# samrussell/zlib-ng

Measured on AMD Instinct MI355X. Metric: GB/s input throughput (adler32, crc32, deflate lvl6, inflate) @1/2/4/8 GPU vs CPU ref, higher is better.
Workload: dtype u8; 1 GPU; configs[1]: crc32 + adler32 over a 1024 MiB synthetic buffer per GPU, HBM-resident, fused single pass + on-device combine; bytes_per_gpu=1073741824, parallelism=single, rehearsal_same_gpu=False

## Files before the change

zlib-ng_amd/csrc/checksum.hip:

```cpp
#include "checksum_kernel.h"

#include <atomic>

namespace zr {

static std::atomic<int> g_reserved_cus{0};

static int pick_groups(const Context *c, long long nunits) {
    long long g = c->cus - g_reserved_cus.load(std::memory_order_relaxed);
    if (g < 1) g = 1;
    if (g > kMaxGroups) g = kMaxGroups;
    if (nunits < g) g = nunits > 0 ? nunits : 1;
    return (int)g;
}

void checksum_reset_reserved_cus() { g_reserved_cus.store(0, std::memory_order_relaxed); }

int launch_checksum(bool do_adler, bool do_crc, uint32_t adler, uint32_t crc, const void *d_buf, void *d_dst,
                    size_t len, uint32_t *d_out_adler, uint32_t *d_out_crc, hipStream_t stream,
                    const uint32_t *d_seed_adler, const uint32_t *d_seed_crc) {
    Context *c = ctx();
    if (!c) {
        set_error("zng_rocm_init() has not succeeded");
        return ZNG_ROCM_ENODEV;
    }
    DeviceGuard dev;
    if ((!d_buf && len) || (do_adler && !d_out_adler) || (do_crc && !d_out_crc)) {
        set_error("null device pointer");
        return ZNG_ROCM_EINVAL;
    }
    if (len >> 34) {
        set_error("length above 16 GiB per call is not supported");
        return ZNG_ROCM_EINVAL;
    }
    Workspace *ws = workspace_for(stream);
    if (!ws) return ZNG_ROCM_ENOMEM;

    const uintptr_t p = (uintptr_t)d_buf;
    const uintptr_t a0 = p & ~(uintptr_t)15;
    const uintptr_t tail_base = (p + len) & ~(uintptr_t)15;
    const bool copy = d_dst != nullptr;
    if (copy && (((uintptr_t)d_dst ^ p) & 15)) {
        set_error("fold_copy needs src and dst with the same address mod 16");
        return ZNG_ROCM_EINVAL;
    }

    StreamArgs sa;
    sa.a0 = (const uint8_t *)a0;
    sa.dst0 = copy ? (uint8_t *)d_dst - (p - a0) : nullptr;
    sa.n = (long long)len;
    sa.body = (long long)(tail_base - a0);
    sa.nunits = (sa.body + kUnitBytes - 1) / kUnitBytes;
    sa.head = (int)(p - a0);
    sa.tail = (int)((p + len) - tail_base);
    sa.phase_stamps = nullptr;
    for (int k = 0; k < 4; ++k)
        for (int i = 0; i < 8; ++i) {
            sa.bits.stride[k][i] = c->host_tables.stride_tab[k][1u << i];
            sa.bits.x32[k][i] = c->host_tables.x32_tab[k][1u << i];
        }

    FinalArgs fa;
    fa.tail_base = (const uint8_t *)tail_base;
    fa.tail_dst = copy ? (uint8_t *)d_dst + (tail_base - p) : nullptr;
    fa.n = sa.n;
    fa.nunits = sa.nunits;
    fa.tail_lo = sa.body == 0 ? sa.head : 0;
    fa.tail_hi = sa.tail;
    if (len == 0) fa.tail_lo = fa.tail_hi = 0;
    fa.adler_seed = adler;
    fa.crc_seed = crc;
    fa.crc_len_pow = do_crc ? xpow_bytes(c->host_tables.pow_tab, (uint64_t)len) : 0u;
    fa.adler_seed_ptr = d_seed_adler;
    fa.crc_seed_ptr = d_seed_crc;
    fa.do_adler = do_adler;
    fa.do_crc = do_crc;

    const int groups = pick_groups(c, sa.nunits);
    fa.groups = groups;
    if (sa.nunits > 0) {
        dim3 grid(groups), block(kWgThreads);
#define ZR_LAUNCH(A, C, K) \
        ZR_LAUNCH_TRACED((stream_kernel<A, C, K>), grid, block, stream, sa, c->tables, ws->partials)
        if (copy) {
            if (do_adler && do_crc) ZR_LAUNCH(true, true, true);
            else if (do_adler) ZR_LAUNCH(true, false, true);
            else ZR_LAUNCH(false, true, true);
        } else {
            if (do_adler && do_crc) ZR_LAUNCH(true, true, false);
            else if (do_adler) ZR_LAUNCH(true, false, false);
            else ZR_LAUNCH(false, true, false);
        }
#undef ZR_LAUNCH
        ZR_HIP(hipGetLastError());
    } else {
        ZR_HIP(hipMemsetAsync(ws->partials, 0, sizeof(Partial) * groups, stream));
    }
    hipLaunchKernelGGL(finalize_kernel, dim3(1), dim3(256), 0, stream, fa, c->tables, ws->partials,
                       d_out_adler, d_out_crc);
    ZR_HIP(hipGetLastError());
    return ZNG_ROCM_OK;
}

int launch_checksum_batch_device(bool do_adler, bool do_crc, const StreamArgs *d_messages, const FinalArgs *d_finals,
                                 Partial *d_part, size_t rows, uint32_t *d_out2, hipStream_t stream) {
    Context *c = ctx();
    if (!c) return ZNG_ROCM_ENODEV;
    if (!rows) return ZNG_ROCM_OK;
    for (size_t first = 0; first < rows; first += 32768) {
        const size_t n = rows - first < 32768 ? rows - first : 32768;
        dim3 grid(1, (unsigned)n), block(kWgThreads);
        if (do_adler && do_crc)
            ZR_LAUNCH_TRACED((stream_kernel_batch<true, true>), grid, block, stream, d_messages + first, c->tables, d_part + first);
        else if (do_adler)
            ZR_LAUNCH_TRACED((stream_kernel_batch<true, false>), grid, block, stream, d_messages + first, c->tables, d_part + first);
        else
            ZR_LAUNCH_TRACED((stream_kernel_batch<false, true>), grid, block, stream, d_messages + first, c->tables, d_part + first);
        ZR_HIP(hipGetLastError());
        hipLaunchKernelGGL(finalize_kernel_batch, dim3((unsigned)n), dim3(256), 0, stream, d_finals + first, c->tables,
                           d_part + first, d_out2 + 2 * first);
        ZR_HIP(hipGetLastError());
    }
    return ZNG_ROCM_OK;
}

}

using namespace zr;

extern "C" {

int zng_rocm_adler32_dev(uint32_t adler, const void *d_buf, size_t len, uint32_t *d_out, void *stream) {
    return launch_checksum(true, false, adler, 0, d_buf, nullptr, len, d_out, nullptr, (hipStream_t)stream);
}

int zng_rocm_crc32_dev(uint32_t crc, const void *d_buf, size_t len, uint32_t *d_out, void *stream) {
    return launch_checksum(false, true, 0, crc, d_buf, nullptr, len, nullptr, d_out, (hipStream_t)stream);
}

int zng_rocm_adler32_crc32_dev(uint32_t adler, uint32_t crc, const void *d_buf, size_t len, uint32_t *d_out2,
                               void *stream) {
    if (!d_out2) return ZNG_ROCM_EINVAL;
    return launch_checksum(true, true, adler, crc, d_buf, nullptr, len, d_out2, d_out2 + 1, (hipStream_t)stream);
}

int zng_rocm_fold_copy_dev(int which, uint32_t adler, uint32_t crc, void *d_dst, const void *d_src, size_t len,
                           uint32_t *d_out2, void *stream) {
    if (which < 1 || which > 3 || !d_out2 || (!d_dst && len)) return ZNG_ROCM_EINVAL;
    if (len == 0) d_dst = nullptr;
    return launch_checksum((which & 1) != 0, (which & 2) != 0, adler, crc, d_src, d_dst, len, d_out2, d_out2 + 1,
                           (hipStream_t)stream);
}

int zng_rocm_reserve_cus(int n) {
    Context *c = ctx();
    if (!c) {
        set_error("zng_rocm_init() has not succeeded");
        return ZNG_ROCM_ENODEV;
    }
    if (n < 0 || n >= c->cus) return ZNG_ROCM_EINVAL;
    g_reserved_cus.store(n, std::memory_order_relaxed);
    return ZNG_ROCM_OK;
}

int zng_rocm_checksums_dev(int which, const zng_rocm_check_job *jobs, size_t njobs, uint32_t *d_out2, void *stream) {
    Context *c = ctx();
    if (!c) {
        set_error("zng_rocm_init() has not succeeded");
        return ZNG_ROCM_ENODEV;
    }
    if (!njobs) return ZNG_ROCM_OK;
    if (which < 1 || which > 3 || !jobs || !d_out2) return ZNG_ROCM_EINVAL;
    const bool do_adler = (which & 1) != 0, do_crc = (which & 2) != 0;
    hipStream_t st = (hipStream_t)stream;
    DeviceGuard dev;
    Workspace *ws = workspace_for(st);
    if (!ws) return ZNG_ROCM_ENOMEM;
    std::lock_guard<std::mutex> use(ws->mu);
    size_t max_units = 1;
    for (size_t i = 0; i < njobs; ++i) {
        if ((!jobs[i].buf && jobs[i].len) || (jobs[i].len >> 34)) {
            set_error("job %zu: null buffer or more than 16 GiB", i);
            return ZNG_ROCM_EINVAL;
        }
        const size_t u = (size_t)((jobs[i].len + 15 + kUnitBytes) / kUnitBytes);
        if (u > max_units) max_units = u;
    }
    size_t G = (max_units + 1023) / 1024;
    if (G > 16) G = 16;
    constexpr size_t kRows = 32768;
    const size_t per = sizeof(StreamArgs) + sizeof(FinalArgs);
    const size_t rows_max = njobs < kRows ? njobs : kRows;
    uint8_t *d_msg = nullptr, *h_msg = nullptr;
    Partial *d_part = nullptr;
    if (int rc = scratch_reserve(ws, kScrCheckMessages, rows_max * per, false, (void **)&d_msg)) return rc;
    if (int rc = scratch_reserve(ws, kScrCheckPartials, rows_max * G * sizeof(Partial), false, (void **)&d_part)) return rc;
    for (size_t first = 0; first < njobs; first += kRows) {
        const size_t rows = njobs - first < kRows ? njobs - first : kRows;
        if (int rc = host_tables_acquire(ws)) return rc;
        if (int rc = scratch_reserve(ws, kScrCheckMessagesHost, rows_max * per, true, (void **)&h_msg)) return rc;
        StreamArgs *sa = reinterpret_cast<StreamArgs *>(h_msg);
        FinalArgs *fa = reinterpret_cast<FinalArgs *>(h_msg + rows * sizeof(StreamArgs));
        for (size_t r = 0; r < rows; ++r) {
            const zng_rocm_check_job &j = jobs[first + r];
            const uintptr_t p = (uintptr_t)j.buf;
            const uintptr_t a0 = p & ~(uintptr_t)15;
            const uintptr_t tail_base = (p + j.len) & ~(uintptr_t)15;
            StreamArgs &s = sa[r];
            s.a0 = (const uint8_t *)a0;
            s.dst0 = nullptr;
            s.n = (long long)j.len;
            s.body = (long long)(tail_base - a0);
            s.nunits = (s.body + kUnitBytes - 1) / kUnitBytes;
            s.head = (int)(p - a0);
            s.tail = (int)((p + j.len) - tail_base);
            s.phase_stamps = nullptr;
            for (int k = 0; k < 4; ++k)
                for (int i = 0; i < 8; ++i) {
                    s.bits.stride[k][i] = c->host_tables.stride_tab[k][1u << i];
                    s.bits.x32[k][i] = c->host_tables.x32_tab[k][1u << i];
                }
            FinalArgs &f = fa[r];
            f.tail_base = (const uint8_t *)tail_base;
            f.tail_dst = nullptr;
            f.n = s.n;
            f.nunits = s.nunits;
            f.tail_lo = s.body == 0 ? s.head : 0;
            f.tail_hi = s.tail;
            if (j.len == 0) f.tail_lo = f.tail_hi = 0;
            f.groups = (int)G;
            f.adler_seed = j.adler;
            f.crc_seed = j.crc;
            f.crc_len_pow = do_crc ? xpow_bytes(c->host_tables.pow_tab, (uint64_t)j.len) : 0u;
            f.adler_seed_ptr = nullptr;
            f.crc_seed_ptr = nullptr;
            f.do_adler = do_adler;
            f.do_crc = do_crc;
        }
        ZR_HIP(hipMemcpyAsync(d_msg, h_msg, rows * per, hipMemcpyHostToDevice, st));
        if (int rc = host_tables_release(ws, st)) return rc;
        const StreamArgs *d_sa = reinterpret_cast<const StreamArgs *>(d_msg);
        const FinalArgs *d_fa = reinterpret_cast<const FinalArgs *>(d_msg + rows * sizeof(StreamArgs));
        dim3 grid((unsigned)G, (unsigned)rows), block(kWgThreads);
        if (do_adler && do_crc) ZR_LAUNCH_TRACED((stream_kernel_batch<true, true>), grid, block, st, d_sa, c->tables, d_part);
        else if (do_adler) ZR_LAUNCH_TRACED((stream_kernel_batch<true, false>), grid, block, st, d_sa, c->tables, d_part);
        else ZR_LAUNCH_TRACED((stream_kernel_batch<false, true>), grid, block, st, d_sa, c->tables, d_part);
        ZR_HIP(hipGetLastError());
        hipLaunchKernelGGL(finalize_kernel_batch, dim3((unsigned)rows), dim3(256), 0, st, d_fa, c->tables, d_part,
                           d_out2 + 2 * first);
        ZR_HIP(hipGetLastError());
    }
    return ZNG_ROCM_OK;
}

}
```

zlib-ng_amd/csrc/checksum_kernel.h:

```cpp
#pragma once
#include "context.h"
#include "checksum_args.h"

namespace zr {

typedef uint32_t u32x4_t __attribute__((ext_vector_type(4)));

__device__ __forceinline__ void st_stream(uint8_t *p, uint4 v) {
    u32x4_t x = {v.x, v.y, v.z, v.w};
    __builtin_nontemporal_store(x, reinterpret_cast<u32x4_t *>(p));
}

__device__ __forceinline__ uint4 ld_stream(const uint8_t *p) {
#ifdef ZR_EXPERIMENT_PLAIN_LOADS
    const u32x4_t v = *reinterpret_cast<const u32x4_t *>(p);
#else
    const u32x4_t v = __builtin_nontemporal_load(reinterpret_cast<const u32x4_t *>(p));
#endif
    return make_uint4(v.x, v.y, v.z, v.w);
}

__device__ __forceinline__ void lds_barrier() {
    __builtin_amdgcn_fence(__ATOMIC_RELEASE, "workgroup", "local");
    __builtin_amdgcn_s_barrier();
    __builtin_amdgcn_fence(__ATOMIC_ACQUIRE, "workgroup", "local");
}

__device__ __forceinline__ uint4 mask_low_bytes(uint4 v, int k) {
    uint32_t w[4] = {v.x, v.y, v.z, v.w};
#pragma unroll
    for (int i = 0; i < 4; ++i) {
        int kk = k - 4 * i;
        if (kk >= 4) w[i] = 0;
        else if (kk > 0) w[i] &= 0xffffffffu << (8 * kk);
    }
    return make_uint4(w[0], w[1], w[2], w[3]);
}

__device__ __forceinline__ uint32_t braid_step(const uint32_t *lut, uint32_t rep, uint32_t s, uint32_t w) {
    uint32_t r0 = lut[(((s)       & 0xffu) << 5) + rep];
    uint32_t r1 = lut[(1u << 13) + (((s >> 8)  & 0xffu) << 5) + rep];
    uint32_t r2 = lut[(2u << 13) + (((s >> 16) & 0xffu) << 5) + rep];
    uint32_t r3 = lut[(3u << 13) + (((s >> 24)       ) << 5) + rep];
    return r0 ^ r1 ^ r2 ^ r3 ^ w;
}

__device__ __forceinline__ uint32_t xor3(uint32_t a, uint32_t b, uint32_t c) {
    return __builtin_amdgcn_bitop3_b32(a, b, c, 0x96);
}
__device__ __forceinline__ uint32_t and_xor(uint32_t a, uint32_t b, uint32_t c) {
    return __builtin_amdgcn_bitop3_b32(a, b, c, 0x6a);
}

typedef const __attribute__((address_space(3))) uint32_t *lds_u32_ptr;
template <int K>
__device__ __forceinline__ void put_index_byte(uint32_t &addr, uint32_t s) {
    if constexpr (K == 0) asm("v_mov_b32_sdwa %0, %1 dst_sel:BYTE_1 dst_unused:UNUSED_PRESERVE src0_sel:BYTE_0" : "+v"(addr) : "v"(s));
    if constexpr (K == 1) asm("v_mov_b32_sdwa %0, %1 dst_sel:BYTE_1 dst_unused:UNUSED_PRESERVE src0_sel:BYTE_1" : "+v"(addr) : "v"(s));
    if constexpr (K == 2) asm("v_mov_b32_sdwa %0, %1 dst_sel:BYTE_1 dst_unused:UNUSED_PRESERVE src0_sel:BYTE_2" : "+v"(addr) : "v"(s));
    if constexpr (K == 3) asm("v_mov_b32_sdwa %0, %1 dst_sel:BYTE_1 dst_unused:UNUSED_PRESERVE src0_sel:BYTE_3" : "+v"(addr) : "v"(s));
}
struct BraidAddr {
    uint32_t a0, a1, a2, a3;
};
__device__ __forceinline__ uint32_t braid_step_bytes(BraidAddr &A, uint32_t s, uint32_t w) {
    put_index_byte<0>(A.a0, s);
    const uint32_t r0 = *(lds_u32_ptr)(uintptr_t)A.a0;
    put_index_byte<1>(A.a1, s);
    const uint32_t r1 = *(lds_u32_ptr)(uintptr_t)A.a1;
    put_index_byte<2>(A.a2, s);
    const uint32_t r2 = *(lds_u32_ptr)(uintptr_t)A.a2;
    put_index_byte<3>(A.a3, s);
    const uint32_t r3 = *(lds_u32_ptr)(uintptr_t)A.a3;
    return xor3(xor3(r0, r1, r2), r3, w);
}

template <bool XOR>
__device__ __forceinline__ uint32_t wave_reduce(uint32_t v) {
    auto op = [](uint32_t a, uint32_t b) { return XOR ? (a ^ b) : (a + b); };
    v = op(v, (uint32_t)__builtin_amdgcn_mov_dpp((int)v, 0xB1, 0xf, 0xf, true));
    v = op(v, (uint32_t)__builtin_amdgcn_mov_dpp((int)v, 0x4E, 0xf, 0xf, true));
    v = op(v, (uint32_t)__builtin_amdgcn_mov_dpp((int)v, 0x141, 0xf, 0xf, true));
    v = op(v, (uint32_t)__builtin_amdgcn_mov_dpp((int)v, 0x140, 0xf, 0xf, true));
    return op(op((uint32_t)__builtin_amdgcn_readlane((int)v, 0), (uint32_t)__builtin_amdgcn_readlane((int)v, 16)),
              op((uint32_t)__builtin_amdgcn_readlane((int)v, 32), (uint32_t)__builtin_amdgcn_readlane((int)v, 48)));
}

__device__ __forceinline__ uint32_t mul_by_rows(const uint4 *rows, int stride, int idx, uint32_t r) {
    uint32_t acc = 0;
#pragma unroll
    for (int kq = 0; kq < 8; ++kq) {
        const uint4 a = rows[kq * stride + idx];
        acc = and_xor((uint32_t)__builtin_amdgcn_sbfe((int)r, 31 - 4 * kq, 1), a.x, acc);
        acc = and_xor((uint32_t)__builtin_amdgcn_sbfe((int)r, 30 - 4 * kq, 1), a.y, acc);
        acc = and_xor((uint32_t)__builtin_amdgcn_sbfe((int)r, 29 - 4 * kq, 1), a.z, acc);
        acc = and_xor((uint32_t)__builtin_amdgcn_sbfe((int)r, 28 - 4 * kq, 1), a.w, acc);
    }
    return acc;
}

constexpr int kVarBothBuffers = 1;
constexpr int kVarFoldX32     = 2;
constexpr int kVarEarlyPow    = 4;
#ifdef ZR_CRC_VARIANTS
constexpr int kVarNoReplicate = 16;
constexpr int kVarNoMultiply  = 32;
#else
constexpr int kVarNoReplicate = 0, kVarNoMultiply = 0;
#endif
constexpr int kVarBuildTables = 64;
constexpr int kVarLdsBarrier  = 128;
constexpr int kVarByteAddr    = 1024;
constexpr int kVarDirectImage = 2048;
constexpr int kVarTreeEpilogue = 4096;
constexpr int kVarWavePrio    = 8192;
constexpr int kVarEarlyRows   = 768;
constexpr int kCrcVariant = kVarFoldX32 | kVarBuildTables | kVarLdsBarrier | kVarByteAddr | kVarDirectImage | kVarTreeEpilogue;

template <bool DO_ADLER, bool DO_CRC, bool COPY, int V, bool PROFILE, int UNROLL>
__device__ __forceinline__ void stream_body(const StreamArgs &args, const DeviceTables *__restrict__ tabs,
                                            Partial *__restrict__ partials, const long long G, const long long g) {
#ifndef ZR_CRC_VARIANTS
    static_assert(V == kCrcVariant, "the product instantiates the one tuned variant; the others are for tools/micro/crc_phases.hip");
#endif
    __shared__ __attribute__((aligned(65536))) uint32_t lut[DO_CRC ? 4 * 256 * 32 : 32];
    __shared__ uint32_t stage[DO_CRC ? 4 * 256 + 256 + 4 * 256 : 4];
    __shared__ uint32_t red[3][kWgThreads / 64];
    constexpr bool TREE = (V & kVarTreeEpilogue) != 0;
    __shared__ uint4 tree_rows[(DO_CRC && TREE) ? 640 : 1];

    const int t = threadIdx.x;
    const uint32_t rep = t & 31;
    auto stamp = [&](int k) {
        if constexpr (PROFILE) {
            if (t == 0) args.phase_stamps[8 * g + k] = wall_clock64();
        }
    };
    stamp(0);
    if constexpr ((V & kVarWavePrio) != 0) {
        const int wv = __builtin_amdgcn_readfirstlane(t >> 6);
        if (wv >= 12) __builtin_amdgcn_s_setprio(3);
        else if (wv >= 8) __builtin_amdgcn_s_setprio(2);
        else if (wv >= 4) __builtin_amdgcn_s_setprio(1);
    }

    const long long q = args.nunits / G, r = args.nunits % G;
    const long long u_lo = g * q + (g < r ? g : r);
    const long long u_hi = u_lo + q + (g < r ? 1 : 0);

    long long off = args.body - (args.nunits - u_lo) * (long long)kUnitBytes + (long long)t * kPieceBytes;

    const bool head_unit = u_lo < u_hi && u_lo == 0;
    const long long groups = (u_hi - u_lo - (head_unit ? 1 : 0)) / UNROLL;
    const long long gstride = (long long)UNROLL * kUnitBytes;
    uint4 bufA[UNROLL], bufB[UNROLL];
    auto request = [&](uint4 (&buf)[UNROLL], long long at) {
#pragma unroll
        for (int j = 0; j < UNROLL; ++j) buf[j] = ld_stream(args.a0 + at + (long long)j * kUnitBytes);
    };
    const long long first_at = off + (head_unit ? (long long)kUnitBytes : 0ll);
    bool b_requested = false;
    uint32_t group_w0 = 0, group_w1 = 0;
    uint32_t part[32];
    uint4 tree_row = make_uint4(0, 0, 0, 0);
    if constexpr (DO_CRC) {
        const unsigned long long k_after = (unsigned long long)(args.nunits - u_hi);
        if constexpr ((V & kVarBuildTables) != 0) {
            constexpr int early = (V & kVarEarlyRows) == 0 ? UNROLL : ((V & kVarEarlyRows) >> 8) - 1;
            if (groups > 0) {
#pragma unroll
                for (int j = 0; j < early; ++j) bufA[j] = ld_stream(args.a0 + first_at + (long long)j * kUnitBytes);
            }
            if constexpr ((V & kVarBothBuffers) != 0 && early == UNROLL) {
                if (groups > 1) {
                    request(bufB, first_at + gstride);
                    b_requested = true;
                }
            }
            group_w0 = tabs->unit_pow[0][k_after & 1023u];
            group_w1 = tabs->unit_pow[1][(k_after >> 10) & 1023u];
            if constexpr (TREE) tree_row = *reinterpret_cast<const uint4 *>(tabs->tree_pp[t]);
            if constexpr ((V & kVarEarlyPow) != 0) {
#pragma unroll
                for (int k = 0; k < 32; ++k) part[k] = tabs->lane_pow[k][t];
            }
            const int k = __builtin_amdgcn_readfirstlane(t >> 8);
            const uint32_t e = (uint32_t)t & 255u;
            if constexpr ((V & kVarDirectImage) != 0) {
                static_assert((V & kVarDirectImage) == 0 || ((V & kVarByteAddr) != 0 && (V & kVarFoldX32) != 0),
                              "direct image: byte-addressed layout and x^32 fold only");
                uint32_t m[7];
#pragma unroll
                for (int b = 0; b < 7; ++b) m[b] = (uint32_t)__builtin_amdgcn_sbfe((int)((uint32_t)t >> 3), b, 1);
#pragma unroll
                for (int j = 0; j < 4; ++j) {
                    uint32_t v = 0;
#pragma unroll
                    for (int b = 0; b < 7; ++b) v = and_xor(m[b], args.bits.stride[j][b], v);
#pragma unroll
                    for (int h = 0; h < 2; ++h) {
                        const uint32_t vv = h ? v ^ args.bits.stride[j][7] : v;
                        const int slot = (j >> 1) * 512 + ((h * 128 + (t >> 3)) << 1) + (j & 1);
                        reinterpret_cast<uint4 *>(lut)[slot * 8 + (t & 7)] = make_uint4(vv, vv, vv, vv);
                    }
                }
                uint32_t xv = 0;
#pragma unroll
                for (int i = 0; i < 8; ++i) xv = and_xor((uint32_t)__builtin_amdgcn_sbfe((int)e, i, 1), args.bits.x32[k][i], xv);
                stage[1280 + t] = xv;
            } else {
                uint32_t sv = 0, xv = 0;
#pragma unroll
                for (int i = 0; i < 8; ++i) {
                    const uint32_t m = 0u - ((e >> i) & 1u);
                    sv ^= args.bits.stride[k][i] & m;
                    xv ^= args.bits.x32[k][i] & m;
                }
                stage[t] = sv;
                stage[1280 + t] = xv;
                if (t < 256) {
                    uint32_t r = e;
#pragma unroll
                    for (int i = 0; i < 8; ++i) r = (r >> 1) ^ (kCrcPoly & (0u - (r & 1u)));
                    stage[1024 + t] = r;
                }
            }
        } else {
            uint4 tab = make_uint4(0, 0, 0, 0);
            if (t < 256) {
                tab = reinterpret_cast<const uint4 *>(&tabs->stride_tab[0][0])[t];
            } else if (t < 320) {
                tab = reinterpret_cast<const uint4 *>(tabs->byte_tab)[t - 256];
            } else if (t < 576) {
                tab = reinterpret_cast<const uint4 *>(&tabs->x32_tab[0][0])[t - 320];
            }
            group_w0 = tabs->unit_pow[0][k_after & 1023u];
            group_w1 = tabs->unit_pow[1][(k_after >> 10) & 1023u];
            if (groups > 0) request(bufA, first_at);
            if constexpr ((V & kVarBothBuffers) != 0) {
                if (groups > 1) {
                    request(bufB, first_at + gstride);
                    b_requested = true;
                }
            }
            if constexpr ((V & kVarEarlyPow) != 0) {
#pragma unroll
                for (int k = 0; k < 32; ++k) part[k] = tabs->lane_pow[k][t];
            }
            if (t < 576) reinterpret_cast<uint4 *>(stage)[t] = tab;
        }
        if constexpr ((V & kVarDirectImage) == 0) {
            if constexpr ((V & kVarLdsBarrier) != 0) lds_barrier();
            else __syncthreads();
        }
        stamp(1);
        if constexpr ((V & kVarNoReplicate) == 0 && (V & kVarDirectImage) == 0) {
#pragma unroll
            for (int i = 0; i < 8; ++i) {
                const uint32_t v = stage[i * 128 + (t >> 3)];
                if constexpr ((V & kVarByteAddr) != 0) {
                    const int slot = (i >> 2) * 512 + (((i & 1) * 128 + (t >> 3)) << 1) + ((i >> 1) & 1);
                    reinterpret_cast<uint4 *>(lut)[slot * 8 + (t & 7)] = make_uint4(v, v, v, v);
                } else {
                    reinterpret_cast<uint4 *>(lut)[i * kWgThreads + t] = make_uint4(v, v, v, v);
                }
            }
        }
        if constexpr ((V & kVarLdsBarrier) != 0) lds_barrier();
        else __syncthreads();
        if constexpr ((V & kVarBuildTables) != 0 && (V & kVarEarlyRows) != 0) {
            constexpr int early = ((V & kVarEarlyRows) >> 8) - 1;
            if (groups > 0) {
#pragma unroll
                for (int j = early; j < UNROLL; ++j) bufA[j] = ld_stream(args.a0 + first_at + (long long)j * kUnitBytes);
            }
            if constexpr ((V & kVarBothBuffers) != 0) {
                if (groups > 1) {
                    request(bufB, first_at + gstride);
                    b_requested = true;
                }
            }
        }
    } else {
        if (groups > 0) request(bufA, first_at);
    }
    stamp(2);

    uint32_t s0 = 0, s1 = 0, s2 = 0, s3 = 0;
    BraidAddr braid_addr;
    if constexpr (DO_CRC && (V & kVarByteAddr) != 0) {
        const uint32_t base = (uint32_t)(uintptr_t)(lds_u32_ptr)lut + rep * 4u;
        if ((base & 0xff00u) != 0) __builtin_trap();
        braid_addr.a0 = base;
        braid_addr.a1 = base + 128u;
        braid_addr.a2 = base + 65536u;
        braid_addr.a3 = base + 65536u + 128u;
    }
    uint32_t S1 = 0, SR = 0, SW = 0;
    uint32_t accA = 0, accB = 0;
    int batch = 0;

    auto fold_adler = [&](long long off_last) {
        const unsigned long long off0 = (unsigned long long)(off_last - (long long)t * kPieceBytes);
        const unsigned long long off0_u = ((unsigned long long)__builtin_amdgcn_readfirstlane((int)(off0 >> 32)) << 32) |
                                          (uint32_t)__builtin_amdgcn_readfirstlane((int)(uint32_t)off0);
        const uint32_t lead0 = (uint32_t)((unsigned long long)(args.n - ((long long)off0_u - args.head) - kPieceBytes) % kAdlerBase);
        const uint32_t back = (uint32_t)t * (uint32_t)kPieceBytes;
        const uint32_t lead = lead0 >= back ? lead0 - back : lead0 + kAdlerBase - back;
        const uint32_t s1m = S1 % kAdlerBase;
        uint32_t v = (lead * s1m) % kAdlerBase;
        v += ((uint32_t)kUnitBytes * (SR % kAdlerBase)) % kAdlerBase;
        v += SW % kAdlerBase;
        accB = (accB + v) % kAdlerBase;
        accA = (accA + s1m) % kAdlerBase;
        S1 = SR = SW = 0;
        batch = 0;
    };

    auto consume = [&](uint4 v) {
        if constexpr (DO_CRC) {
            if constexpr ((V & kVarByteAddr) != 0) {
                s0 = braid_step_bytes(braid_addr, s0, v.x);
                s1 = braid_step_bytes(braid_addr, s1, v.y);
                s2 = braid_step_bytes(braid_addr, s2, v.z);
                s3 = braid_step_bytes(braid_addr, s3, v.w);
            } else {
                s0 = braid_step(lut, rep, s0, v.x);
                s1 = braid_step(lut, rep, s1, v.y);
                s2 = braid_step(lut, rep, s2, v.z);
                s3 = braid_step(lut, rep, s3, v.w);
            }
        }
        if constexpr (DO_ADLER) {
            SR += S1;
            S1 = __builtin_amdgcn_sad_u8(v.x, 0u, S1);
            S1 = __builtin_amdgcn_sad_u8(v.y, 0u, S1);
            S1 = __builtin_amdgcn_sad_u8(v.z, 0u, S1);
            S1 = __builtin_amdgcn_sad_u8(v.w, 0u, S1);
            SW = __builtin_amdgcn_udot4(v.x, 0x0D0E0F10u, SW, false);
            SW = __builtin_amdgcn_udot4(v.y, 0x090A0B0Cu, SW, false);
            SW = __builtin_amdgcn_udot4(v.z, 0x05060708u, SW, false);
            SW = __builtin_amdgcn_udot4(v.w, 0x01020304u, SW, false);
        }
    };

    long long u = u_lo;
    if (u < u_hi && u == 0) {
        uint4 v = make_uint4(0, 0, 0, 0);
        if (off >= 0) {
            v = *reinterpret_cast<const uint4 *>(args.a0 + off);
            if (off == 0 && args.head) v = mask_low_bytes(v, args.head);
            if constexpr (COPY) {
                if (off == 0 && args.head) {
                    for (int j = args.head; j < 16; ++j) args.dst0[j] = args.a0[j];
                } else {
                    *reinterpret_cast<uint4 *>(args.dst0 + off) = v;
                }
            }
        }
        consume(v);
        if constexpr (DO_ADLER) { batch = 1; }
        off += kUnitBytes;
        ++u;
    }

    constexpr int BATCH_MAX = 240;
    if (groups > 0) {
        auto retire = [&](uint4 (&buf)[UNROLL]) {
            if constexpr (COPY) {
#pragma unroll
                for (int j = 0; j < UNROLL; ++j)
                    st_stream(args.dst0 + off + (long long)j * kUnitBytes, buf[j]);
            }
#pragma unroll
            for (int j = 0; j < UNROLL; ++j) consume(buf[j]);
            off += (long long)UNROLL * kUnitBytes;
            if constexpr (DO_ADLER) {
                batch += UNROLL;
                if (batch >= BATCH_MAX) fold_adler(off - kUnitBytes);
            }
        };
        long long k = 0;
        if (b_requested) {
            __builtin_amdgcn_sched_barrier(0);
            retire(bufA);
            k = 1;
            while (k + 2 < groups) {
                request(bufA, off + gstride);
                __builtin_amdgcn_sched_barrier(0);
                retire(bufB);
                request(bufB, off + gstride);
                __builtin_amdgcn_sched_barrier(0);
                retire(bufA);
                k += 2;
            }
            if (groups - k == 2) {
                request(bufA, off + gstride);
                __builtin_amdgcn_sched_barrier(0);
                retire(bufB);
                retire(bufA);
            } else {
                retire(bufB);
            }
        } else {
            while (k + 2 < groups) {
                request(bufB, off + gstride);
                __builtin_amdgcn_sched_barrier(0);
                retire(bufA);
                request(bufA, off + gstride);
                __builtin_amdgcn_sched_barrier(0);
                retire(bufB);
                k += 2;
            }
            if (groups - k == 2) {
                request(bufB, off + gstride);
                __builtin_amdgcn_sched_barrier(0);
                retire(bufA);
                retire(bufB);
            } else {
                retire(bufA);
            }
        }
        u += groups * UNROLL;
    }
    for (; u < u_hi; ++u) {
        uint4 v = *reinterpret_cast<const uint4 *>(args.a0 + off);
        if constexpr (COPY) *reinterpret_cast<uint4 *>(args.dst0 + off) = v;
        consume(v);
        off += kUnitBytes;
        if constexpr (DO_ADLER) ++batch;
    }
    if constexpr (DO_ADLER) {
        if (batch) fold_adler(off - kUnitBytes);
    }
    stamp(3);

    uint32_t pc = 0;
    if constexpr (DO_CRC) {
        if (u_hi > u_lo) {
            uint32_t r = s0;
            if constexpr ((V & kVarFoldX32) != 0) {
                const uint32_t *xt = stage + 1280;
#pragma unroll
                for (int c = 0; c < 3; ++c) {
                    r = xt[r & 0xffu] ^ xt[256 + ((r >> 8) & 0xffu)] ^ xt[512 + ((r >> 16) & 0xffu)] ^ xt[768 + (r >> 24)];
                    r ^= c == 0 ? s1 : (c == 1 ? s2 : s3);
                }
            } else {
                const uint32_t *bt = stage + 1024;
#pragma unroll
                for (int c = 0; c < 3; ++c) {
#pragma unroll
                    for (int k = 0; k < 4; ++k) r = bt[r & 0xffu] ^ (r >> 8);
                    r ^= c == 0 ? s1 : (c == 1 ? s2 : s3);
                }
            }
            if constexpr ((V & kVarNoMultiply) != 0) {
                pc = r;
            } else if constexpr (TREE) {
                pc = r;
            } else {
                if constexpr ((V & kVarEarlyPow) == 0) {
#pragma unroll
                    for (int k = 0; k < 32; ++k) part[k] = tabs->lane_pow[k][t];
                }
#pragma unroll
                for (int k = 0; k < 32; ++k) pc ^= part[k] & (0u - ((r >> (31 - k)) & 1u));
            }
        }
    }
    const int wave = t >> 6;
    const int lane = t & 63;
    if constexpr (TREE) {
        uint32_t gpp = 0;
        if constexpr (DO_CRC) {
            if (t < 640) tree_rows[t] = tree_row;
            if (wave == 0) {
                gpp = lane < 32 ? group_w0 : group_w1;
                const int steps = lane & 31;
                for (int i = 0; i < 31; ++i) {
                    const uint32_t nx = (gpp >> 1) ^ (kCrcPoly & (0u - (gpp & 1u)));
                    gpp = i < steps ? nx : gpp;
                }
            }
            lds_barrier();
            if constexpr ((V & kVarNoMultiply) == 0) pc = mul_by_rows(tree_rows, 64, lane, pc);
        }
        stamp(4);
        uint32_t wc = 0, wa = 0, wb = 0;
        if constexpr (DO_CRC) wc = wave_reduce<true>(pc);
        if constexpr (DO_ADLER) {
            wa = wave_reduce<false>(accA);
            wb = wave_reduce<false>(accB);
        }
        if (lane == 0) {
            red[0][wave] = wc;
            red[1][wave] = wa;
            red[2][wave] = wb;
        }
        lds_barrier();
        if (wave == 0) {
            uint32_t c = 0, a = 0, b = 0;
            if constexpr (DO_CRC) {
                uint32_t v = lane < 16 ? red[0][lane & 15] : 0u;
                v = mul_by_rows(tree_rows + 512, 16, lane & 15, v);
                c = wave_reduce<true>(v);
                const uint32_t sel = 31u - (uint32_t)(lane & 31);
                c = wave_reduce<true>(lane < 32 ? gpp & (0u - ((c >> sel) & 1u)) : 0u);
                c = wave_reduce<true>(lane >= 32 ? gpp & (0u - ((c >> sel) & 1u)) : 0u);
            }
            if constexpr (DO_ADLER) {
                a = wave_reduce<false>(lane < 16 ? red[1][lane & 15] : 0u);
                b = wave_reduce<false>(lane < 16 ? red[2][lane & 15] : 0u);
            }
            if (lane == 0) {
                Partial pt;
                pt.crc = c;
                pt.a = a % kAdlerBase;
                pt.b = b % kAdlerBase;
                pt.pad = 0;
                partials[g] = pt;
            }
        }
    } else {
        stamp(4);
        uint32_t pa = accA, pb = accB;
#pragma unroll
        for (int m = 32; m >= 1; m >>= 1) {
            if constexpr (DO_CRC) pc ^= __shfl_xor(pc, m, 64);
            if constexpr (DO_ADLER) {
                pa += __shfl_xor(pa, m, 64);
                pb += __shfl_xor(pb, m, 64);
            }
        }
        if ((t & 63) == 0) {
            red[0][wave] = pc;
            red[1][wave] = pa;
            red[2][wave] = pb;
        }
        __syncthreads();
        if (t == 0) {
            uint32_t c = 0;
            unsigned long long a = 0, b = 0;
            for (int w = 0; w < kWgThreads / 64; ++w) {
                c ^= red[0][w];
                a += red[1][w];
                b += red[2][w];
            }
            if constexpr (DO_CRC) {
                const unsigned long long k = (unsigned long long)(args.nunits - u_hi);
                if (c && k) {
                    c = mulmod(c, group_w0);
                    if (k >> 10) c = mulmod(c, group_w1);
                }
            }
            Partial pt;
            pt.crc = c;
            pt.a = (uint32_t)(a % kAdlerBase);
            pt.b = (uint32_t)(b % kAdlerBase);
            pt.pad = 0;
            partials[g] = pt;
        }
    }
    stamp(5);
}

constexpr int kRowsPerBuffer = 1, kRowsPerBufferCopy = 4;
template <bool DO_ADLER, bool DO_CRC, bool COPY, int V = kCrcVariant, bool PROFILE = false,
          int UNROLL = COPY ? kRowsPerBufferCopy : kRowsPerBuffer>
__global__ __launch_bounds__(kWgThreads)
void stream_kernel(StreamArgs args, const DeviceTables *__restrict__ tabs, Partial *__restrict__ partials) {
    stream_body<DO_ADLER, DO_CRC, COPY, V, PROFILE, UNROLL>(args, tabs, partials, gridDim.x, blockIdx.x);
}

template <bool DO_ADLER, bool DO_CRC, int V = kCrcVariant>
__global__ __launch_bounds__(kWgThreads)
void stream_kernel_batch(const StreamArgs *__restrict__ messages, const DeviceTables *__restrict__ tabs,
                         Partial *__restrict__ partials) {
    stream_body<DO_ADLER, DO_CRC, false, V, false, kRowsPerBuffer>(messages[blockIdx.y], tabs, partials + (size_t)blockIdx.y * gridDim.x,
                                                      gridDim.x, blockIdx.x);
}


__device__ __forceinline__
void finalize_body(const FinalArgs &fa, const DeviceTables *__restrict__ tabs, const Partial *__restrict__ partials,
                   uint32_t *__restrict__ out_adler, uint32_t *__restrict__ out_crc) {
    __shared__ uint32_t red[3][4];
    const int t = threadIdx.x;
    const long long G = fa.groups;
    const int ntail = fa.tail_hi - fa.tail_lo;

    uint32_t c = 0;
    unsigned long long a = 0, b = 0;
    for (long long g = t; g < G; g += blockDim.x) {
        Partial p = partials[g];
        c ^= p.crc;
        a += p.a;
        b += p.b;
    }
    uint32_t tc = 0;
    if (t < ntail) {
        uint32_t byte = fa.tail_base[fa.tail_lo + t];
        if (fa.tail_dst) fa.tail_dst[fa.tail_lo + t] = (uint8_t)byte;
        int after = ntail - 1 - t;
        if (fa.do_crc) tc = mulmod(tabs->byte_tab[byte], tabs->pow_tab[after]);
        a += byte;
        b += (unsigned long long)byte * (unsigned)(after + 1);
    }
    __shared__ uint32_t red_t[4];
#pragma unroll
    for (int m = 32; m >= 1; m >>= 1) {
        c ^= __shfl_xor(c, m, 64);
        tc ^= __shfl_xor(tc, m, 64);
        a += __shfl_xor(a, m, 64);
        b += __shfl_xor(b, m, 64);
    }
    if ((t & 63) == 0) {
        red_t[t >> 6] = tc;
        red[0][t >> 6] = c;
        red[1][t >> 6] = (uint32_t)(a % kAdlerBase);
        red[2][t >> 6] = (uint32_t)(b % kAdlerBase);
    }
    __syncthreads();
    if (t == 0) {
        uint32_t cc = red[0][0] ^ red[0][1] ^ red[0][2] ^ red[0][3];
        unsigned long long A = (unsigned long long)red[1][0] + red[1][1] + red[1][2] + red[1][3];
        unsigned long long B = (unsigned long long)red[2][0] + red[2][1] + red[2][2] + red[2][3];
        if (fa.do_adler) {
            const uint32_t seed = fa.adler_seed_ptr ? *fa.adler_seed_ptr : fa.adler_seed;
            unsigned long long s1 = seed & 0xffffu, s2 = (seed >> 16) & 0xffffu;
            unsigned long long n_mod = (unsigned long long)fa.n % kAdlerBase;
            unsigned long long r1 = (s1 + A) % kAdlerBase;
            unsigned long long r2 = (s2 + n_mod * s1 + B) % kAdlerBase;
            *out_adler = (uint32_t)(r1 | (r2 << 16));
        }
        if (fa.do_crc) {
            const uint32_t seed = fa.crc_seed_ptr ? *fa.crc_seed_ptr : fa.crc_seed;
            const uint32_t seed_term = mulmod(~seed, fa.crc_len_pow);
            const uint32_t body = (ntail && cc) ? mulmod(cc, tabs->pow_tab[ntail]) : cc;
            *out_crc = ~(body ^ red_t[0] ^ red_t[1] ^ red_t[2] ^ red_t[3] ^ seed_term);
        }
    }
}

__global__ __launch_bounds__(256)
void finalize_kernel(FinalArgs fa, const DeviceTables *__restrict__ tabs, const Partial *__restrict__ partials,
                     uint32_t *__restrict__ out_adler, uint32_t *__restrict__ out_crc) {
    finalize_body(fa, tabs, partials, out_adler, out_crc);
}

__global__ __launch_bounds__(256)
void finalize_kernel_batch(const FinalArgs *__restrict__ messages, const DeviceTables *__restrict__ tabs,
                           const Partial *__restrict__ partials, uint32_t *__restrict__ out2) {
    const FinalArgs fa = messages[blockIdx.x];
    finalize_body(fa, tabs, partials + (size_t)blockIdx.x * fa.groups, out2 + 2 * (size_t)blockIdx.x,
                  out2 + 2 * (size_t)blockIdx.x + 1);
}


}
```

Before: 6575 GB/s.

## Fuse checksum finalize into stream kernel via last-block ticket combine

Folds the finalize step into the streaming checksum kernel. The last workgroup to finish, found through an atomic ticket, reduces packed per-group partials and writes the final adler/crc. Seed and tail precomputation runs during idle CRC epilogue slots, and the separate finalize launch is dropped when the fused path applies. The non-fused finalize shrinks to one wave. This removes a second kernel launch and its dependency gap, at the cost of atomics and a ticket that must be reset correctly between calls.

```diff
diff --git a/zlib-ng_amd/csrc/checksum.hip b/zlib-ng_amd/csrc/checksum.hip
--- a/zlib-ng_amd/csrc/checksum.hip
+++ b/zlib-ng_amd/csrc/checksum.hip
@@ -13,6 +13,8 @@
     if (nunits < g) g = nunits > 0 ? nunits : 1;
     return (int)g;
 }
+
+constexpr long long kFusedMinUnitsPerGroup = 64;
 
 void checksum_reset_reserved_cus() { g_reserved_cus.store(0, std::memory_order_relaxed); }
 
@@ -76,12 +78,19 @@
     fa.do_adler = do_adler;
     fa.do_crc = do_crc;
 
-    const int groups = pick_groups(c, sa.nunits);
+    const int groups = sa.nunits > 0 ? pick_groups(c, sa.nunits) : 0;
+    const bool fused = groups == 1 || (groups > 1 && sa.nunits >= kFusedMinUnitsPerGroup * groups);
     fa.groups = groups;
     if (sa.nunits > 0) {
         dim3 grid(groups), block(kWgThreads);
+#define ZR_LAUNCH_F(A, C, K, F) \
+        ZR_LAUNCH_TRACED((stream_kernel<A, C, K, kCrcVariant, false, K ? kRowsPerBufferCopy : kRowsPerBuffer, F>), grid, \
+                         block, stream, sa, c->tables, ws->partials, fa, d_out_adler, d_out_crc, ws->acc)
 #define ZR_LAUNCH(A, C, K) \
-        ZR_LAUNCH_TRACED((stream_kernel<A, C, K>), grid, block, stream, sa, c->tables, ws->partials)
+        do { \
+            if (fused) ZR_LAUNCH_F(A, C, K, true); \
+            else ZR_LAUNCH_F(A, C, K, false); \
+        } while (0)
         if (copy) {
             if (do_adler && do_crc) ZR_LAUNCH(true, true, true);
             else if (do_adler) ZR_LAUNCH(true, false, true);
@@ -92,13 +101,14 @@
             else ZR_LAUNCH(false, true, false);
         }
 #undef ZR_LAUNCH
-        ZR_HIP(hipGetLastError());
-    } else {
-        ZR_HIP(hipMemsetAsync(ws->partials, 0, sizeof(Partial) * groups, stream));
-    }
-    hipLaunchKernelGGL(finalize_kernel, dim3(1), dim3(256), 0, stream, fa, c->tables, ws->partials,
-                       d_out_adler, d_out_crc);
-    ZR_HIP(hipGetLastError());
+#undef ZR_LAUNCH_F
+        ZR_HIP(hipGetLastError());
+    }
+    if (!fused) {
+        hipLaunchKernelGGL(finalize_kernel, dim3(1), dim3(64), 0, stream, fa, c->tables, ws->partials, d_out_adler,
+                           d_out_crc);
+        ZR_HIP(hipGetLastError());
+    }
     return ZNG_ROCM_OK;
 }
 
@@ -110,15 +120,13 @@
     for (size_t first = 0; first < rows; first += 32768) {
         const size_t n = rows - first < 32768 ? rows - first : 32768;
         dim3 grid(1, (unsigned)n), block(kWgThreads);
-        if (do_adler && do_crc)
-            ZR_LAUNCH_TRACED((stream_kernel_batch<true, true>), grid, block, stream, d_messages + first, c->tables, d_part + first);
-        else if (do_adler)
-            ZR_LAUNCH_TRACED((stream_kernel_batch<true, false>), grid, block, stream, d_messages + first, c->tables, d_part + first);
-        else
-            ZR_LAUNCH_TRACED((stream_kernel_batch<false, true>), grid, block, stream, d_messages + first, c->tables, d_part + first);
-        ZR_HIP(hipGetLastError());
-        hipLaunchKernelGGL(finalize_kernel_batch, dim3((unsigned)n), dim3(256), 0, stream, d_finals + first, c->tables,
-                           d_part + first, d_out2 + 2 * first);
+#define ZR_LAUNCH(A, C) \
+        ZR_LAUNCH_TRACED((stream_kernel_batch<A, C>), grid, block, stream, d_messages + first, c->tables, d_part + first, \
+                         d_finals + first, d_out2 + 2 * first)
+        if (do_adler && do_crc) ZR_LAUNCH(true, true);
+        else if (do_adler) ZR_LAUNCH(true, false);
+        else ZR_LAUNCH(false, true);
+#undef ZR_LAUNCH
         ZR_HIP(hipGetLastError());
     }
     return ZNG_ROCM_OK;
@@ -242,15 +250,20 @@
         const StreamArgs *d_sa = reinterpret_cast<const StreamArgs *>(d_msg);
         const FinalArgs *d_fa = reinterpret_cast<const FinalArgs *>(d_msg + rows * sizeof(StreamArgs));
         dim3 grid((unsigned)G, (unsigned)rows), block(kWgThreads);
-        if (do_adler && do_crc) ZR_LAUNCH_TRACED((stream_kernel_batch<true, true>), grid, block, st, d_sa, c->tables, d_part);
-        else if (do_adler) ZR_LAUNCH_TRACED((stream_kernel_batch<true, false>), grid, block, st, d_sa, c->tables, d_part);
-        else ZR_LAUNCH_TRACED((stream_kernel_batch<false, true>), grid, block, st, d_sa, c->tables, d_part);
-        ZR_HIP(hipGetLastError());
-        hipLaunchKernelGGL(finalize_kernel_batch, dim3((unsigned)rows), dim3(256), 0, st, d_fa, c->tables, d_part,
-                           d_out2 + 2 * first);
-        ZR_HIP(hipGetLastError());
-    }
-    return ZNG_ROCM_OK;
-}
-
-}
+#define ZR_LAUNCH(A, C) \
+        ZR_LAUNCH_TRACED((stream_kernel_batch<A, C>), grid, block, st, d_sa, c->tables, d_part, d_fa, d_out2 + 2 * first)
+        if (do_adler && do_crc) ZR_LAUNCH(true, true);
+        else if (do_adler) ZR_LAUNCH(true, false);
+        else ZR_LAUNCH(false, true);
+#undef ZR_LAUNCH
+        ZR_HIP(hipGetLastError());
+        if (G > 1) {
+            hipLaunchKernelGGL(finalize_kernel_batch, dim3((unsigned)rows), dim3(64), 0, st, d_fa, c->tables, d_part,
+                               d_out2 + 2 * first);
+            ZR_HIP(hipGetLastError());
+        }
+    }
+    return ZNG_ROCM_OK;
+}
+
+}
diff --git a/zlib-ng_amd/csrc/checksum_kernel.h b/zlib-ng_amd/csrc/checksum_kernel.h
--- a/zlib-ng_amd/csrc/checksum_kernel.h
+++ b/zlib-ng_amd/csrc/checksum_kernel.h
@@ -117,9 +117,9 @@
 constexpr int kVarEarlyRows   = 768;
 constexpr int kCrcVariant = kVarFoldX32 | kVarBuildTables | kVarLdsBarrier | kVarByteAddr | kVarDirectImage | kVarTreeEpilogue;
 
-template <bool DO_ADLER, bool DO_CRC, bool COPY, int V, bool PROFILE, int UNROLL>
-__device__ __forceinline__ void stream_body(const StreamArgs &args, const DeviceTables *__restrict__ tabs,
-                                            Partial *__restrict__ partials, const long long G, const long long g) {
+template <bool DO_ADLER, bool DO_CRC, bool COPY, int V, bool PROFILE, int UNROLL, class Idle>
+__device__ __forceinline__ Partial stream_body(const StreamArgs &args, const DeviceTables *__restrict__ tabs,
+                                               const long long G, const long long g, Idle &&idle) {
 #ifndef ZR_CRC_VARIANTS
     static_assert(V == kCrcVariant, "the product instantiates the one tuned variant; the others are for tools/micro/crc_phases.hip");
 #endif
@@ -131,6 +131,7 @@
 
     const int t = threadIdx.x;
     const uint32_t rep = t & 31;
+    Partial pt = {0u, 0u, 0u, 0u};
     auto stamp = [&](int k) {
         if constexpr (PROFILE) {
             if (t == 0) args.phase_stamps[8 * g + k] = wall_clock64();
@@ -482,6 +483,7 @@
                     const uint32_t nx = (gpp >> 1) ^ (kCrcPoly & (0u - (gpp & 1u)));
                     gpp = i < steps ? nx : gpp;
                 }
+                idle();
             }
             lds_barrier();
             if constexpr ((V & kVarNoMultiply) == 0) pc = mul_by_rows(tree_rows, 64, lane, pc);
@@ -497,6 +499,9 @@
             red[0][wave] = wc;
             red[1][wave] = wa;
             red[2][wave] = wb;
+        }
+        if constexpr (!DO_CRC) {
+            if (wave == 0) idle();
         }
         lds_barrier();
         if (wave == 0) {
@@ -513,14 +518,9 @@
                 a = wave_reduce<false>(lane < 16 ? red[1][lane & 15] : 0u);
                 b = wave_reduce<false>(lane < 16 ? red[2][lane & 15] : 0u);
             }
-            if (lane == 0) {
-                Partial pt;
-                pt.crc = c;
-                pt.a = a % kAdlerBase;
-                pt.b = b % kAdlerBase;
-                pt.pad = 0;
-                partials[g] = pt;
-            }
+            pt.crc = c;
+            pt.a = a % kAdlerBase;
+            pt.b = b % kAdlerBase;
         }
     } else {
         stamp(4);
@@ -554,108 +554,211 @@
                     if (k >> 10) c = mulmod(c, group_w1);
                 }
             }
-            Partial pt;
             pt.crc = c;
             pt.a = (uint32_t)(a % kAdlerBase);
             pt.b = (uint32_t)(b % kAdlerBase);
-            pt.pad = 0;
-            partials[g] = pt;
         }
     }
     stamp(5);
-}
+    return pt;
+}
+
+struct FinalPre {
+    uint32_t x;
+    uint32_t adv;
+    uint32_t byte;
+    uint32_t base_a;
+    uint32_t base_b;
+    int ntail;
+};
+
+__device__ __forceinline__
+FinalPre finalize_pre(const FinalArgs &fa, const DeviceTables *__restrict__ tabs, const bool do_adler, const bool do_crc) {
+    const int lane = threadIdx.x & 63;
+    FinalPre p = {0u, 0u, 0u, 0u, 0u, fa.tail_hi - fa.tail_lo};
+    uint32_t mx = 0, my = 0;
+    uint32_t ta = 0, tb = 0;
+    if (lane < p.ntail) {
+        p.byte = fa.tail_base[fa.tail_lo + lane];
+        const int after = p.ntail - 1 - lane;
+        ta = p.byte;
+        tb = p.byte * (uint32_t)(after + 1);
+        if (do_crc) {
+            mx = tabs->byte_tab[p.byte];
+            my = tabs->pow_tab[after];
+        }
+    }
+    if (do_crc) {
+        if (lane == 32) {
+            const uint32_t seed = fa.crc_seed_ptr ? *fa.crc_seed_ptr : fa.crc_seed;
+            mx = ~seed;
+            my = fa.crc_len_pow;
+        }
+        p.x = wave_reduce<true>(mulmod(mx, my));
+        if (p.ntail) {
+            p.adv = tabs->pow_tab[p.ntail];
+            const int steps = lane & 31;
+            for (int i = 0; i < 31; ++i) {
+                const uint32_t nx = (p.adv >> 1) ^ (kCrcPoly & (0u - (p.adv & 1u)));
+                p.adv = i < steps ? nx : p.adv;
+            }
+        }
+    }
+    if (do_adler) {
+        const uint32_t seed = fa.adler_seed_ptr ? *fa.adler_seed_ptr : fa.adler_seed;
+        const uint32_t s1 = seed & 0xffffu, s2 = (seed >> 16) & 0xffffu;
+        const uint32_t n_mod = (uint32_t)((unsigned long long)fa.n % kAdlerBase);
+        p.base_a = s1 + (p.ntail ? wave_reduce<false>(ta) : 0u);
+        p.base_b = s2 + (n_mod * s1) % kAdlerBase + (p.ntail ? wave_reduce<false>(tb) : 0u);
+    }
+    return p;
+}
+
+template <bool REDUCED>
+__device__ __forceinline__
+void finalize_body(const FinalArgs &fa, const FinalPre &p, uint32_t c, uint32_t a, uint32_t b, const bool do_adler,
+                   const bool do_crc, uint32_t *__restrict__ out_adler, uint32_t *__restrict__ out_crc) {
+    const int lane = threadIdx.x & 63;
+    if (fa.tail_dst && lane < p.ntail) fa.tail_dst[fa.tail_lo + lane] = (uint8_t)p.byte;
+    if (do_adler) {
+        if constexpr (!REDUCED) {
+            a = wave_reduce<false>(a);
+            b = wave_reduce<false>(b);
+        }
+        const uint32_t r1 = (p.base_a + a) % kAdlerBase, r2 = (p.base_b + b) % kAdlerBase;
+        if (lane == 0) *out_adler = r1 | (r2 << 16);
+    }
+    if (do_crc) {
+        if constexpr (!REDUCED) c = wave_reduce<true>(c);
+        if (p.ntail) {
+            const uint32_t sel = 31u - (uint32_t)(lane & 31);
+            c = wave_reduce<true>(lane < 32 ? p.adv & (0u - ((c >> sel) & 1u)) : 0u);
+        }
+        if (lane == 0) *out_crc = ~(c ^ p.x);
+    }
+}
+
+__device__ __forceinline__ bool seeds_in_arguments(const FinalArgs &fa) { return !fa.adler_seed_ptr && !fa.crc_seed_ptr; }
+
+__device__ __forceinline__ void add_stored_partials(const Partial *__restrict__ partials, long long G, uint32_t &c,
+                                                    uint32_t &a, uint32_t &b) {
+    for (long long g = threadIdx.x & 63; g < G; g += 64) {
+        const Partial p = partials[g];
+        c ^= p.crc;
+        a += p.a;
+        b += p.b;
+    }
+}
+
+typedef __attribute__((address_space(1))) unsigned long long gu64;
+typedef __attribute__((address_space(1))) uint32_t gu32;
 
 constexpr int kRowsPerBuffer = 1, kRowsPerBufferCopy = 4;
+
 template <bool DO_ADLER, bool DO_CRC, bool COPY, int V = kCrcVariant, bool PROFILE = false,
-          int UNROLL = COPY ? kRowsPerBufferCopy : kRowsPerBuffer>
+          int UNROLL = COPY ? kRowsPerBufferCopy : kRowsPerBuffer, bool FUSED = false>
 __global__ __launch_bounds__(kWgThreads)
-void stream_kernel(StreamArgs args, const DeviceTables *__restrict__ tabs, Partial *__restrict__ partials) {
-    stream_body<DO_ADLER, DO_CRC, COPY, V, PROFILE, UNROLL>(args, tabs, partials, gridDim.x, blockIdx.x);
+void stream_kernel(StreamArgs args, const DeviceTables *__restrict__ tabs, Partial *partials, FinalArgs fa,
+                   uint32_t *__restrict__ out_adler, uint32_t *__restrict__ out_crc, uint32_t *ticket) {
+    if constexpr (!FUSED) {
+        const Partial pt = stream_body<DO_ADLER, DO_CRC, COPY, V, PROFILE, UNROLL>(args, tabs, gridDim.x, blockIdx.x, [] {});
+        if (threadIdx.x == 0) partials[blockIdx.x] = pt;
+    } else {
+        static_assert((V & kVarTreeEpilogue) != 0, "the fused form needs the partial uniform over wave 0");
+        const bool early = seeds_in_arguments(fa);
+        FinalPre pre = {0u, 0u, 0u, 0u, 0u, 0};
+        const Partial pt = stream_body<DO_ADLER, DO_CRC, COPY, V, PROFILE, UNROLL>(args, tabs, gridDim.x, blockIdx.x, [&] {
+            if (early) pre = finalize_pre(fa, tabs, DO_ADLER, DO_CRC);
+        });
+        if (threadIdx.x >= 64) return;
+        const int lane = threadIdx.x;
+        const uint32_t G = gridDim.x;
+        if (G == 1) {
+            if (!early) pre = finalize_pre(fa, tabs, DO_ADLER, DO_CRC);
+            finalize_body<true>(fa, pre, pt.crc, pt.a, pt.b, DO_ADLER, DO_CRC, out_adler, out_crc);
+        } else {
+            gu64 *slots = (gu64 *)partials;
+            uint32_t arrived = 0;
+            if (lane == 0) {
+                __hip_atomic_store(slots + blockIdx.x,
+                                   (unsigned long long)pt.crc | ((unsigned long long)(pt.a | (pt.b << 16)) << 32),
+                                   __ATOMIC_RELAXED, __HIP_MEMORY_SCOPE_AGENT);
+                asm volatile("s_waitcnt vmcnt(0)" ::: "memory");
+                arrived = __hip_atomic_fetch_add((gu32 *)ticket, 1u, __ATOMIC_RELAXED, __HIP_MEMORY_SCOPE_AGENT);
+            }
+            arrived = (uint32_t)__builtin_amdgcn_readfirstlane((int)arrived);
+            if (arrived != G - 1) return;
+            __builtin_amdgcn_fence(__ATOMIC_ACQUIRE, "wavefront");
+            unsigned long long w[4];
+#pragma unroll
+            for (int j = 0; j < 4; ++j) {
+                const uint32_t g = (uint32_t)lane + 64u * j;
+                w[j] = __hip_atomic_load(slots + (g < G ? g : G - 1), __ATOMIC_RELAXED, __HIP_MEMORY_SCOPE_AGENT);
+            }
+            if (!early) pre = finalize_pre(fa, tabs, DO_ADLER, DO_CRC);
+            uint32_t c = 0, a = 0, b = 0;
+            auto add = [&](unsigned long long v) {
+                c ^= (uint32_t)v;
+                a += (uint32_t)(v >> 32) & 0xffffu;
+                b += (uint32_t)(v >> 48);
+            };
+#pragma unroll
+            for (int j = 0; j < 4; ++j) {
+                asm volatile("" : "+v"(w[j]));
+                if ((uint32_t)lane + 64u * j < G) add(w[j]);
+            }
+            for (uint32_t g = 256u + (uint32_t)lane; g < G; g += 64u)
+                add(__hip_atomic_load(slots + g, __ATOMIC_RELAXED, __HIP_MEMORY_SCOPE_AGENT));
+            finalize_body<false>(fa, pre, c, a, b, DO_ADLER, DO_CRC, out_adler, out_crc);
+            if (lane == 0) __hip_atomic_store((gu32 *)ticket, 0u, __ATOMIC_RELAXED, __HIP_MEMORY_SCOPE_AGENT);
+        }
+        if constexpr (PROFILE) {
+            if (lane == 0) args.phase_stamps[8 * blockIdx.x + 6] = wall_clock64();
+        }
+    }
 }
 
 template <bool DO_ADLER, bool DO_CRC, int V = kCrcVariant>
 __global__ __launch_bounds__(kWgThreads)
 void stream_kernel_batch(const StreamArgs *__restrict__ messages, const DeviceTables *__restrict__ tabs,
-                         Partial *__restrict__ partials) {
-    stream_body<DO_ADLER, DO_CRC, false, V, false, kRowsPerBuffer>(messages[blockIdx.y], tabs, partials + (size_t)blockIdx.y * gridDim.x,
-                                                      gridDim.x, blockIdx.x);
-}
-
-
-__device__ __forceinline__
-void finalize_body(const FinalArgs &fa, const DeviceTables *__restrict__ tabs, const Partial *__restrict__ partials,
-                   uint32_t *__restrict__ out_adler, uint32_t *__restrict__ out_crc) {
-    __shared__ uint32_t red[3][4];
-    const int t = threadIdx.x;
-    const long long G = fa.groups;
-    const int ntail = fa.tail_hi - fa.tail_lo;
-
-    uint32_t c = 0;
-    unsigned long long a = 0, b = 0;
-    for (long long g = t; g < G; g += blockDim.x) {
-        Partial p = partials[g];
-        c ^= p.crc;
-        a += p.a;
-        b += p.b;
-    }
-    uint32_t tc = 0;
-    if (t < ntail) {
-        uint32_t byte = fa.tail_base[fa.tail_lo + t];
-        if (fa.tail_dst) fa.tail_dst[fa.tail_lo + t] = (uint8_t)byte;
-        int after = ntail - 1 - t;
-        if (fa.do_crc) tc = mulmod(tabs->byte_tab[byte], tabs->pow_tab[after]);
-        a += byte;
-        b += (unsigned long long)byte * (unsigned)(after + 1);
-    }
-    __shared__ uint32_t red_t[4];
-#pragma unroll
-    for (int m = 32; m >= 1; m >>= 1) {
-        c ^= __shfl_xor(c, m, 64);
-        tc ^= __shfl_xor(tc, m, 64);
-        a += __shfl_xor(a, m, 64);
-        b += __shfl_xor(b, m, 64);
-    }
-    if ((t & 63) == 0) {
-        red_t[t >> 6] = tc;
-        red[0][t >> 6] = c;
-        red[1][t >> 6] = (uint32_t)(a % kAdlerBase);
-        red[2][t >> 6] = (uint32_t)(b % kAdlerBase);
-    }
-    __syncthreads();
-    if (t == 0) {
-        uint32_t cc = red[0][0] ^ red[0][1] ^ red[0][2] ^ red[0][3];
-        unsigned long long A = (unsigned long long)red[1][0] + red[1][1] + red[1][2] + red[1][3];
-        unsigned long long B = (unsigned long long)red[2][0] + red[2][1] + red[2][2] + red[2][3];
-        if (fa.do_adler) {
-            const uint32_t seed = fa.adler_seed_ptr ? *fa.adler_seed_ptr : fa.adler_seed;
-            unsigned long long s1 = seed & 0xffffu, s2 = (seed >> 16) & 0xffffu;
-            unsigned long long n_mod = (unsigned long long)fa.n % kAdlerBase;
-            unsigned long long r1 = (s1 + A) % kAdlerBase;
-            unsigned long long r2 = (s2 + n_mod * s1 + B) % kAdlerBase;
-            *out_adler = (uint32_t)(r1 | (r2 << 16));
-        }
-        if (fa.do_crc) {
-            const uint32_t seed = fa.crc_seed_ptr ? *fa.crc_seed_ptr : fa.crc_seed;
-            const uint32_t seed_term = mulmod(~seed, fa.crc_len_pow);
-            const uint32_t body = (ntail && cc) ? mulmod(cc, tabs->pow_tab[ntail]) : cc;
-            *out_crc = ~(body ^ red_t[0] ^ red_t[1] ^ red_t[2] ^ red_t[3] ^ seed_term);
-        }
-    }
-}
-
-__global__ __launch_bounds__(256)
+                         Partial *__restrict__ partials, const FinalArgs *__restrict__ finals, uint32_t *__restrict__ out2) {
+    static_assert((V & kVarTreeEpilogue) != 0, "finalizing in place needs the partial uniform over wave 0");
+    const bool solo = gridDim.x == 1;
+    const FinalArgs fa = finals[blockIdx.y];
+    const bool early = solo && seeds_in_arguments(fa);
+    FinalPre pre = {0u, 0u, 0u, 0u, 0u, 0};
+    const Partial pt = stream_body<DO_ADLER, DO_CRC, false, V, false, kRowsPerBuffer>(messages[blockIdx.y], tabs, gridDim.x, blockIdx.x, [&] {
+        if (early) pre = finalize_pre(fa, tabs, fa.do_adler != 0, fa.do_crc != 0);
+    });
+    if (threadIdx.x >= 64) return;
+    if (solo) {
+        if (!early) pre = finalize_pre(fa, tabs, fa.do_adler != 0, fa.do_crc != 0);
+        finalize_body<true>(fa, pre, pt.crc, pt.a, pt.b, fa.do_adler != 0, fa.do_crc != 0, out2 + 2 * (size_t)blockIdx.y,
+                            out2 + 2 * (size_t)blockIdx.y + 1);
+    } else if (threadIdx.x == 0) {
+        partials[(size_t)blockIdx.y * gridDim.x + blockIdx.x] = pt;
+    }
+}
+
+__global__ __launch_bounds__(64)
 void finalize_kernel(FinalArgs fa, const DeviceTables *__restrict__ tabs, const Partial *__restrict__ partials,
                      uint32_t *__restrict__ out_adler, uint32_t *__restrict__ out_crc) {
-    finalize_body(fa, tabs, partials, out_adler, out_crc);
-}
-
-__global__ __launch_bounds__(256)
+    const FinalPre pre = finalize_pre(fa, tabs, fa.do_adler != 0, fa.do_crc != 0);
+    uint32_t c = 0, a = 0, b = 0;
+    add_stored_partials(partials, fa.groups, c, a, b);
+    finalize_body<false>(fa, pre, c, a, b, fa.do_adler != 0, fa.do_crc != 0, out_adler, out_crc);
+}
+
+__global__ __launch_bounds__(64)
 void finalize_kernel_batch(const FinalArgs *__restrict__ messages, const DeviceTables *__restrict__ tabs,
                            const Partial *__restrict__ partials, uint32_t *__restrict__ out2) {
     const FinalArgs fa = messages[blockIdx.x];
-    finalize_body(fa, tabs, partials + (size_t)blockIdx.x * fa.groups, out2 + 2 * (size_t)blockIdx.x,
-                  out2 + 2 * (size_t)blockIdx.x + 1);
-}
-
-
-}
+    const FinalPre pre = finalize_pre(fa, tabs, fa.do_adler != 0, fa.do_crc != 0);
+    uint32_t c = 0, a = 0, b = 0;
+    add_stored_partials(partials + (size_t)blockIdx.x * fa.groups, fa.groups, c, a, b);
+    finalize_body<false>(fa, pre, c, a, b, fa.do_adler != 0, fa.do_crc != 0, out2 + 2 * (size_t)blockIdx.x,
+                         out2 + 2 * (size_t)blockIdx.x + 1);
+}
+
+
+}
```

Result: no change. 6631 GB/s (median of 6 runs) (+0.9%).
